# liayan/Legion-1

Measured on AMD Instinct MI355X. Metric: sampled edges/s + feature GB/s, 3-hop GraphSAGE ogbn-papers100M at 1/2/4/8 GPU, higher is better.
Workload: dtype int32 ids / f32 rows (verbatim copy)

## Files before the change

### legion-1_amd/csrc/internal.h

```cpp
#pragma once
#include <hip/hip_runtime.h>
#include <cstdint>
#include <cstdio>
#include <cstdlib>
#include <iostream>
#include <string>
#include <vector>

#include "../../include/legion_amd.h"
#include "audit.h"

namespace legion {

void report_error(const char* file, int line, const char* msg, bool hip_failure);
bool error_pending();
bool error_is_fatal();
int64_t ipc_max_bytes();
bool ipc_size_ok(int64_t bytes, const char* who);
bool ipc_export_ok(const void* ptr, const char* who);
int64_t shard_chunk_bytes();
inline void check(hipError_t e, const char* file, int line)
{
    if (e != hipSuccess) report_error(file, line, hipGetErrorString(e), true);
}
#define HIP_CHECK(expr) ::legion::check((expr), __FILE__, __LINE__)
#define HIP_CHECK_LAST() ::legion::check(hipGetLastError(), __FILE__, __LINE__)
#define LEGION_ARG_ERROR(msg) ::legion::report_error(__FILE__, __LINE__, (msg), false)

std::ostream& log_out();
FILE* log_file();

int physical_device(int logical);
bool is_remote_device(int logical);
struct DeviceGuard {
    int prev = -1, prev_logical = -1;
    explicit DeviceGuard(int logical);
    ~DeviceGuard();
};

int chunk_shift(int64_t unit_bytes, int min_shift);
inline int chunk_count(int64_t n, int shift) { return n > 0 ? (int)(((n - 1) >> shift) + 1) : 1; }
template <typename T>
struct ChunkList {
    std::vector<T*> chunks;
    bool imported = false;
    T* at(int q) const { return q >= 0 && q < (int)chunks.size() ? chunks[q] : nullptr; }
    bool complete(size_t n) const { for (T* p : chunks) if (!p) return false; return chunks.size() == n; }
    void release();
    int export_chunk(int dev, int q, void* handle64, const char* who) const;
    int import_chunk(int q, const void* handle64, int64_t floor_bytes, int open_dev, const char* who);
};
template <typename T> void upload_table(int viewer, const std::vector<T*>& h, T**& tab, bool realloc, const char* what);

typedef unsigned long long pos_t;
constexpr int kPosShift = 32;
constexpr uint32_t kProvisional = 0x80000000u, kPosValueMask = 0x7FFFFFFFu;
constexpr uint32_t kEpochTop = 0xFFFFFFFFu, kSerialLimit = 0xFFFFFFF0u;
__host__ __device__ inline pos_t pos_entry(uint32_t epoch, uint32_t value) { return ((pos_t)epoch << kPosShift) | (pos_t)value; }
#ifndef LEGION_KTILE
#define LEGION_KTILE 1024
#endif
constexpr int kTile = LEGION_KTILE;
constexpr int kBlock = 256;
static_assert(kTile >= kBlock && kTile <= 2048 && (kTile & (kTile - 1)) == 0, "LEGION_KTILE: a power of two in [256, 2048] (k_sample stages 16 bytes of row descriptor per slot in static LDS)");
#ifndef LEGION_NARROW_SLOTS
#define LEGION_NARROW_SLOTS (256 * 1024)
#endif
constexpr int kTileNarrow = kBlock;
constexpr int64_t kNarrowSlots = LEGION_NARROW_SLOTS;
static_assert(kTileNarrow <= kTile, "one pow_tab of kTile entries serves both tile sizes");
constexpr int64_t sampler_tile_of(int64_t slots_bound) { return slots_bound <= kNarrowSlots ? kTileNarrow : kTile; }
constexpr int64_t sampler_max_tiles(int64_t max_slots)
{
    const int64_t wide = (max_slots + kTile - 1) / kTile, narrow_slots = max_slots < kNarrowSlots ? max_slots : kNarrowSlots;
    const int64_t narrow = (narrow_slots + kTileNarrow - 1) / kTileNarrow;
    return wide > narrow ? wide : narrow;
}
constexpr int kDistinctMaxFanout = 64;
constexpr int32_t kSamplingReplace = 0, kSamplingDistinct = 1, kSamplingWeighted = 2;
struct AliasEntry { uint32_t thr; int32_t alias_id; };
static_assert(sizeof(AliasEntry) == 8, "one 8-byte probe per weighted draw");
constexpr int32_t kAliasHubDegree = 256;
constexpr int kMaxChunks = 2048;
static_assert(kMaxChunks % kBlock == 0 && kMaxChunks >= 256 * 8, "kMaxChunks: a multiple of the workgroup size, >= 256 CUs x 8 workgroups");
constexpr int ilog2_c(int v) { return v <= 1 ? 0 : 1 + ilog2_c(v >> 1); }
constexpr int kMaxParts = LEGION_MAX_DEVICE;

struct ServeModes {
    bool agg_last_hop = false;
    int32_t agg_norm = 0;
    int32_t sampling = 0;
    bool seeded = false;
    uint32_t seed = 0;
    int32_t lp_draw = 0;
    bool weighted_distinct = false;
    bool operator==(const ServeModes& o) const { return agg_last_hop == o.agg_last_hop && agg_norm == o.agg_norm && sampling == o.sampling && seeded == o.seeded && seed == o.seed && lp_draw == o.lp_draw && weighted_distinct == o.weighted_distinct; }
};
bool serve_modes_from_env(ServeModes& m, std::string& why);
bool serve_modes_resolve_lp_draw(ServeModes& m, bool lp_lists, int32_t raw_batch_size, std::string& why);
bool serve_modes_fit_fanout(const ServeModes& m, const int32_t* fanout, int32_t hops, std::string& why);
void runner_set_lists_verbatim(Runner* r, bool verbatim);
void ipc_env_publish_modes(IPCEnv* e, const ServeModes& m);

constexpr int kModes = 3;
static_assert(LEGION_TRAINMODE == 0 && LEGION_VALIDMODE == 1 && LEGION_TESTMODE == 2, "seed sets are indexed by mode");
struct BuildInfoSeedFields {
    const int32_t* LegionBuildInfo::*num;
    const int32_t* const* LegionBuildInfo::*ids;
    const int32_t* const* LegionBuildInfo::*labels;
};
constexpr BuildInfoSeedFields kBuildInfoSeeds[kModes] = {
    {&LegionBuildInfo::training_set_num, &LegionBuildInfo::training_set_ids, &LegionBuildInfo::training_labels},
    {&LegionBuildInfo::validation_set_num, &LegionBuildInfo::validation_set_ids, &LegionBuildInfo::validation_labels},
    {&LegionBuildInfo::testing_set_num, &LegionBuildInfo::testing_set_ids, &LegionBuildInfo::testing_labels}};

constexpr uint32_t kP31 = 2147483647u;
constexpr uint32_t kA = 48271u;

__host__ __device__ inline uint32_t mulmod31(uint32_t a, uint32_t b)
{
    uint64_t p = (uint64_t)a * (uint64_t)b;
    uint32_t r = (uint32_t)(p & kP31) + (uint32_t)(p >> 31);
    r = (r & kP31) + (r >> 31);
    return r >= kP31 ? r - kP31 : r;
}

__host__ __device__ inline uint32_t powmod31(uint32_t base, uint64_t e)
{
    uint32_t r = 1;
    while (e) {
        if (e & 1) r = mulmod31(r, base);
        base = mulmod31(base, base);
        e >>= 1;
    }
    return r;
}

__host__ __device__ inline uint32_t mix32(uint32_t z)
{
    z ^= z >> 16; z *= 0x7feb352du; z ^= z >> 15; z *= 0x846ca68bu; z ^= z >> 16;
    return z;
}
constexpr uint32_t kShuffleTag = 0x53485546u, kDrawTag = 0x44524157u, kGolden = 0x9E3779B9u;
constexpr uint32_t kLpPosTag = 0x4C50504Fu, kLpNegTag = 0x4C504E45u;
__host__ __device__ inline uint32_t seeded_shuffle_key(uint32_t seed, uint32_t round) { return mix32(mix32(seed ^ kShuffleTag) ^ round); }
__host__ __device__ inline uint32_t seeded_draw_key(uint32_t seed, uint32_t round) { return mix32(mix32(seed ^ kDrawTag) ^ round); }
__host__ __device__ inline uint32_t seeded_draw_word(uint32_t seeded, uint32_t draw_key, int32_t counter) { return seeded ? mix32(draw_key ^ (uint32_t)counter) : 0u; }
__host__ __device__ inline uint32_t seeded_stream_seed(uint32_t w) { return 1u + w % 2147483646u; }
__host__ __device__ inline uint32_t seeded_perm(uint32_t g, uint32_t n, uint32_t ks)
{
    if (n <= 1) return g;
    uint32_t b = 0;
    while (b < 32 && ((n - 1) >> b)) b++;
    const uint32_t h = (b + 1) >> 1, m = (1u << h) - 1u;
    uint32_t rk[4];
    for (uint32_t q = 0; q < 4; q++) rk[q] = mix32(ks + q * kGolden);
    uint32_t x = g;
    do {
        uint32_t L = x >> h, R = x & m;
        for (uint32_t q = 0; q < 4; q++) { const uint32_t t = L ^ (mix32(R ^ rk[q]) & m); L = R; R = t; }
        x = (L << h) | R;
    } while (x >= n);
    return x;
}

struct FastDiv {
    uint32_t d = 1, m = 0, s = 0;
    FastDiv() = default;
    explicit FastDiv(uint32_t div);
};

struct CsrTables {
    const int64_t* indptr;
    const int32_t* indices;
    const int64_t* const* frag_indptr;
    const int32_t* const* frag_indices;
    int32_t ip_nch, ix_nch, row_shift, edge_shift;
    int32_t partition_count;
    const int8_t* topo_owner;
    const int32_t* topo_row;
};

struct BatchCtl {
    int32_t counter;
    uint32_t epoch;
    uint32_t draw;
    uint32_t seeded;
    uint32_t draw_key;
};

struct HopState {
    int32_t edge_base, node_base, n_edges, n_nodes, in_off, n_in, slots, pad;
};

struct SamplerBuffers {
    int32_t* sampled_ids;
    int32_t* agg_src_ids;
    int32_t* agg_src_off;
    int32_t* agg_dst_off;
    int32_t* nc;
    int32_t* ec;
    pos_t* pos_map;
    const BatchCtl* ctl;
    int32_t* cand;
    int32_t* aux;
    int32_t* aux_next;
    int32_t next_count;
    int32_t aux_cap;
    int32_t ids_cap;
    int32_t V;
    bool aux_prepared;
    int32_t* tile_edge;
    int32_t* tile_node;
    int2* tile_pre;
    int2* chunk_tot;
    HopState* hop_state;
    unsigned long long* edge_access_time;
};

struct LpDrawArgs {
    int32_t k = 0;
    int32_t V = 0;
    CsrTables csr = {};
};
void launch_seed(hipStream_t s, int32_t* batch_ids, int32_t* labels, int32_t batch_size, int32_t size, int32_t counter,
                 const int32_t* all_ids, const int32_t* all_labels, int32_t total_cap, pos_t* pos_map,
                 uint32_t epoch, BatchCtl* ctl, bool self_driven, int32_t* nc, int32_t* ec, int32_t* aux_next,
                 int32_t f_next, int32_t aux_cap, uint32_t seeded = 0, uint32_t draw_key = 0, const LpDrawArgs* lp = nullptr);
void launch_set_cursor(hipStream_t s, BatchCtl* ctl, int32_t counter, uint32_t epoch, uint32_t seeded = 0, uint32_t draw_key = 0);
void launch_shuffle_seeds(hipStream_t s, const int32_t* ids, const int32_t* labels, int32_t n, uint32_t ks, int32_t* out_ids, int32_t* out_labels);
void launch_shuffle_triples(hipStream_t s, const int32_t* ids, const int32_t* labels, int32_t n, int32_t k, uint32_t ks, int32_t* out_ids, int32_t* out_labels);
void launch_advance(hipStream_t s, BatchCtl* ctl);
int sampler_cu_count();
void warm_static_tables();
void launch_sample_hop(hipStream_t s, const CsrTables& csr, const SamplerBuffers& b, int32_t count, int32_t op_id,
                       int32_t hops, int32_t slots_bound, bool is_presc, int32_t sampling = kSamplingReplace, const AliasEntry* alias = nullptr,
                       const float* weights = nullptr);
void launch_check_weights(hipStream_t s, const float* w, int64_t E, unsigned long long* bad);
void launch_build_alias(hipStream_t s, const int64_t* indptr, const int32_t* indices, const float* w, int32_t V, int64_t E, double* p, AliasEntry* table);
void launch_weighted_probe(hipStream_t s, const int32_t* row, const int32_t* hop, const int32_t* slot, const int32_t* deg, const uint32_t* word,
                           int32_t* k, uint32_t* ub, int32_t n);
void launch_weighted_distinct_probe(hipStream_t s, const int32_t* row, const int32_t* hop, const int32_t* col, const uint32_t* word, const float* w,
                                    uint32_t* u, double* key, int32_t n);
void launch_find_feat(hipStream_t s, const int32_t* sampled_ids, int32_t* cache_offset, const int32_t* nc,
                      int32_t op_id, const int32_t* feat_map, int32_t bound);
void launch_find_topo(hipStream_t s, const int32_t* input_ids, int8_t* part_index, int32_t* part_offset,
                      int32_t batch_size, const int8_t* topo_owner, const int32_t* topo_row);
struct GatherArgs {
    const float* table;
    const float* const* shard_tab;
    int32_t chunk_shift, nchunks;
    const int32_t* feat_map;
    const float** row_ptr;
    int32_t cache_capacity;
    int32_t F;
    int32_t table_pitch, shard_pitch;
    int32_t total_num_nodes;
    const int32_t* sampled_ids;
    const int32_t* nc;
    float* dst;
    int32_t off_idx, size_idx;
    int32_t dst_rows;
    int32_t* rows_seen;
    int32_t* hit_stats;
    int32_t rows_hint;
    bool table_on_host;
    bool row_ptr_ready;
};
void launch_gather(hipStream_t s, const GatherArgs& a, int32_t rows_bound);
void launch_gather_sum(hipStream_t s, const GatherArgs& a, const int32_t* cand, int32_t cand_cap, const int32_t* ec, int32_t hops,
                       int32_t f, int32_t runs_bound, const float* wdraw = nullptr);
struct AggNormArgs {
    const int32_t* nc;
    const int32_t* ec;
    int32_t hops, f;
    const int32_t* cand;
    int32_t cand_cap;
    const int32_t* src_off;
    int32_t ids_cap;
    int32_t* out_deg;
    int32_t* chunk_cnt;
    float* wdraw;
};
void launch_agg_norm_weights(hipStream_t s, const AggNormArgs& a, int32_t slots_bound, int32_t edges_bound);
constexpr int kRowsSeenAll = LEGION_MAX_HOPS + 1;
constexpr int kRowsSeenAggIn = LEGION_MAX_HOPS + 2;
constexpr int kRowsSeenAggRuns = LEGION_MAX_HOPS + 3;
constexpr int kRowsSeenWords = LEGION_MAX_HOPS + 4;
void launch_exchange_plan(hipStream_t s, const GatherArgs& g, int32_t me, int32_t Kg, int32_t* slot, int32_t* counts,
                          int32_t* req_row, int32_t* req_dst, int32_t rows_bound);
void launch_exchange_rows(hipStream_t s, bool scatter, const float* const* shard_chunks, int32_t chunk_shift, const int32_t* list,
                          int32_t n, int32_t F, int32_t shard_pitch, const float* in, float* out, int32_t out_rows);
void launch_hotness(hipStream_t s, const int32_t* ids, const int32_t* nc, int32_t hops, unsigned long long* access,
                    int32_t* max_ids, int32_t bound);
void launch_rng_probe(hipStream_t s, const int32_t* idx, const int32_t* deg, int32_t* k, int32_t n);
void launch_distinct_probe(hipStream_t s, const int32_t* row, const int32_t* hop, const int32_t* deg, int32_t f, int32_t* pos, int32_t n);
void launch_seeded_rng_probe(hipStream_t s, uint32_t w, const int32_t* idx, const int32_t* deg, int32_t* k, int32_t n);
void launch_seeded_distinct_probe(hipStream_t s, uint32_t w, const int32_t* row, const int32_t* hop, const int32_t* deg, int32_t f, int32_t* pos, int32_t n);
void launch_perm_probe(hipStream_t s, uint32_t ks, int32_t n, int32_t* out);
void launch_lp_draw_probe(hipStream_t s, uint32_t w, const int32_t* src, const int32_t* deg, int32_t V, int32_t* rho, int32_t* neg, int32_t n);
void launch_aggregate_access(hipStream_t s, unsigned long long* agg, const unsigned long long* add, int32_t n);
void launch_iota(hipStream_t s, int32_t* out, int32_t n);
void launch_build_feat_map(hipStream_t s, int32_t* feat_map, const int32_t* QF, int32_t capacity, int32_t Kg, int32_t V);
void launch_build_topo_map(hipStream_t s, int8_t* owner, int32_t* row, const int32_t* QT, int32_t capacity, int32_t Kg,
                           int32_t Ki, int32_t V);
void launch_fill_i32(hipStream_t s, int32_t* p, int32_t v, int64_t n);
void launch_fill_i8(hipStream_t s, int8_t* p, int8_t v, int64_t n);
void launch_feat_fill_up(hipStream_t s, int32_t row0, int32_t rows, int32_t F, int32_t chunk_pitch, int32_t table_pitch, float* chunk,
                         const float* table, const int32_t* QF, int32_t Kg, int32_t Ki, int32_t V);
void launch_copy_rows_pitched(hipStream_t s, float* dst, int32_t dst_pitch, const float* src, int32_t src_pitch, int32_t F, int64_t rows);
void launch_neighbor_count(hipStream_t s, const int32_t* QT, int32_t Kg, int32_t Ki, int32_t capacity, int32_t V,
                           const int64_t* indptr, int64_t* count_out);
void launch_topo_fill_up(hipStream_t s, const int32_t* QT, int32_t Kg, int32_t Ki, int32_t capacity, int32_t V,
                         const int64_t* indptr, const int32_t* indices, const int64_t* frag_indptr,
                         int32_t* const* frag_chunks, int32_t edge_shift);
void launch_chunk_ends(hipStream_t s, const int64_t* frag_indptr, int32_t capacity, int32_t edge_shift, int32_t nch, int64_t* ends);
void launch_edge_mem(hipStream_t s, const int32_t* order, uint64_t* edge_mem, int32_t V, const int64_t* indptr);
void launch_topo_transactions(hipStream_t s, const int32_t* order, const uint64_t* hot, uint64_t* out, int32_t V, const int64_t* indptr);
void sort_by_hotness_desc(hipStream_t s, unsigned long long* keys, int32_t* ids, int32_t n);
void inclusive_scan_u64(hipStream_t s, const uint64_t* in, uint64_t* out, int32_t n);
void inclusive_scan_i64(hipStream_t s, const int64_t* in, int64_t* out, int32_t n);

}

struct PeerExchange;
struct GPUMemoryPool {
    int32_t pipeline_depth = LEGION_PIPELINE_DEPTH;
    int32_t current_pipe = 0, iter = 0, mode = 0, op_id = 0;
    int32_t device_id = -1;
    bool owns_scratch = false;
    int32_t V = 0, batch_size = 0, hops = 0, num_ids = 0;
    int32_t fanout[LEGION_MAX_HOPS] = {0};
    int32_t max_slots = 0, max_tiles = 0;
    int32_t feature_rows = 0;
    legion::pos_t* pos_map = nullptr;
    uint32_t batch_serial = 0;
    legion::BatchCtl* ctl = nullptr;
    int32_t* rows_seen = nullptr;
    int32_t* rows_seen_dev = nullptr;
    bool capturing = false;
    bool ctl_synced = false;
    int32_t ctl_counter = 0;
    int32_t* cand = nullptr;
    legion::ServeModes modes;
    std::vector<int32_t*> cand_pipe;
    int32_t sampled_hop = 0;
    bool sampled_presc = false;
    uint32_t levels_gathered = 0;
    uint32_t round = 0;
    int32_t* shuf_ids = nullptr;
    int32_t* shuf_labels = nullptr;
    int32_t shuf_cap = 0, shuf_n = 0;
    const int32_t* shuf_src = nullptr;
    bool shuf_valid = false, shuf_file_order = false;
    bool seed_reads_shuffle = false;
    GPUGraphStorage* lp_graph = nullptr;
    std::vector<int32_t*> agg_out_deg, agg_chunk_cnt;
    std::vector<float*> agg_wdraw;
    int32_t* aux2[2] = {nullptr, nullptr};
    int32_t aux_ready_hop = 0, aux_ready_count = 0;
    int32_t* tile_edge = nullptr;
    int32_t* tile_node = nullptr;
    int2* tile_pre = nullptr;
    int2* chunk_tot = nullptr;
    legion::HopState* hop_state = nullptr;
    int32_t* cache_search_buffer = nullptr;
    const float** row_ptr = nullptr;
    PeerExchange* peer_exchange = nullptr;
    int32_t* agg_src_ids = nullptr;
    int8_t* tmp_part_ind = nullptr;
    int32_t* tmp_part_off = nullptr;
    std::vector<float*> float_features;
    std::vector<int32_t*> labels, node_counter, edge_counter, sampled_ids, agg_src_off, agg_dst_off;
    int32_t bound_n = 0;
    int32_t bound_nodes = 0;
    int32_t level_bound[LEGION_MAX_HOPS + 1] = {0};
    explicit GPUMemoryPool(int32_t depth);
};
namespace legion {
bool pool_apply_modes(GPUMemoryPool* p, const ServeModes& wanted, const char* who);
}

struct GPUGraphStorage {
    int32_t partition_count = 0;
    int32_t node_num = 0;
    int64_t edge_num = 0, cache_edge_num = 0;
    int64_t* csr_node_index_cpu = nullptr;
    int32_t* csr_dst_node_ids_cpu = nullptr;
    std::vector<int64_t*> replica_indptr;
    std::vector<int32_t*> replica_indices;
    std::vector<legion::AliasEntry*> alias;
    std::vector<float*> weights;
    bool retain_weights = false;
    int32_t csr_location = LEGION_LOC_HOST_PINNED;
    bool owns_csr = false;
    struct Fragment {
        int32_t rows = 0;
        int64_t edges = 0;
        legion::ChunkList<int64_t> ip;
        legion::ChunkList<int32_t> ix;
        bool complete = false;
    };
    std::vector<Fragment> frag;
    int32_t row_shift = 27, edge_shift = 28;
    std::vector<std::vector<bool>> view;
    std::vector<void**> d_frag_tab;
    int32_t ip_nch = 1, ix_nch = 1;
};

struct GPUNodeStorage {
    int32_t partition_count = 0, total_num_nodes = 0, float_attr_len = 0;
    float* float_attrs = nullptr;
    int32_t float_attr_pitch = 0;
    std::vector<float*> replica_attrs;
    int32_t replica_pitch = 0;
    int32_t features_location = LEGION_LOC_HOST_PINNED;
    bool owns_features = false;
    struct SeedSet { int32_t num = 0; int32_t* ids = nullptr; int32_t* labels = nullptr; };
    std::vector<SeedSet> seeds[legion::kModes];
    const SeedSet& seed_set(int32_t mode, int32_t p) const
    {
        static const SeedSet none;
        return mode >= 0 && mode < legion::kModes && p >= 0 && p < (int32_t)seeds[mode].size() ? seeds[mode][p] : none;
    }
};

struct CacheController {
    int32_t device_idx = 0, device_count = 1, total_num_nodes = 0, train_step = 0;
    unsigned long long* node_access_time = nullptr;
    unsigned long long* edge_access_time = nullptr;
    int32_t iter = 0, max_ids = 0;
    int32_t* d_max_ids = nullptr;
    int32_t node_capacity = 0, edge_capacity = 0;
    int32_t* feat_map = nullptr;
    int8_t* topo_owner = nullptr;
    int32_t* topo_row = nullptr;
    int32_t* d_global_count = nullptr;
    int32_t find_iter = 0;
    int32_t* hit_stats = nullptr;
    int32_t* hit_stats_dev = nullptr;
    hipEvent_t hit_ev[2] = {nullptr, nullptr};
    bool hit_ev_armed[2] = {false, false};
    int32_t hit_samples = 0;
    double last_hit_rate = -1.0;
};

struct GPUCache {
    int32_t device_count = 0;
    std::vector<CacheController*> ctl;
    std::vector<int32_t*> QF, QT;
    std::vector<unsigned long long*> AF, AT;
    int Kc = 1, Kg = 1;
    std::vector<int32_t> node_capacity, edge_capacity;
    std::vector<double> alpha;
    int64_t cache_memory = 0;
    int32_t int_attr_len = 0, float_attr_len = 0, train_step = 0;
    std::vector<legion::ChunkList<float>> shards;
    std::vector<float**> d_shard_tab;
    std::vector<int32_t> chunk_shift, nchunks;
    int32_t shard_pitch = 0;
    bool is_presc = true;
    bool capacity_forced = false;
    int32_t forced_node_capacity = 0, forced_edge_capacity = 0;
};
```

### legion-1_amd/csrc/sampler.hip

```cpp
#include "internal.h"
#include "draws.h"
#include "launch.h"
#include <mutex>

#include "audit_hooks.h"

namespace legion {

__device__ inline int32_t lp_pos(const CsrTables& c, uint32_t w, uint32_t i, int32_t src)
{
    const int64_t* ip = c.indptr + src;
    const int32_t* rowp;
    const int8_t owner = c.topo_owner ? c.topo_owner[src] : (int8_t)-1;
    int64_t start;
    if (owner >= 0) {
        const int32_t row = c.topo_row[src];
        ip = c.frag_indptr[owner * c.ip_nch + (row >> c.row_shift)] + (row & ((1 << c.row_shift) - 1));
        start = ip[0];
        rowp = c.frag_indices[owner * c.ix_nch + (int32_t)(start >> c.edge_shift)] + (start & ((1ll << c.edge_shift) - 1));
    } else {
        start = ip[0];
        rowp = c.indices + start;
    }
    const int32_t d = (int32_t)(ip[1] - start);
    if (d <= 0) return src;
    const int32_t pos = rowp[lp_rho(w, i, src, d)];
    return pos < 0 ? src : pos;
}

template <bool SELF, bool LP>
__global__ __launch_bounds__(kBlock) void k_seed(int32_t* __restrict__ batch_ids, int32_t* __restrict__ labels,
                                                 int32_t batch_size, int32_t size, int32_t counter,
                                                 const int32_t* __restrict__ all_ids,
                                                 const int32_t* __restrict__ all_labels, int32_t total_cap,
                                                 pos_t* __restrict__ pos_map, uint32_t epoch,
                                                 BatchCtl* __restrict__ ctl, int32_t* __restrict__ nc,
                                                 int32_t* __restrict__ ec, int32_t* __restrict__ aux_next,
                                                 int32_t f_next, int32_t aux_cap, uint32_t seeded, uint32_t draw_key, LpDrawArgs lp)
{
    int32_t idx = threadIdx.x + blockDim.x * blockIdx.x;
    if (SELF) {
        counter = ctl->counter;
        epoch = ctl->epoch;
        const int64_t done = (int64_t)batch_size * counter;
        size = (done + batch_size >= total_cap) ? (int32_t)max((int64_t)0, min((int64_t)batch_size, (int64_t)total_cap - done)) : batch_size;
    } else if (idx == 0) {
        ctl->counter = counter;
        ctl->epoch = epoch;
        ctl->draw = seeded_draw_word(seeded, draw_key, counter);
        ctl->seeded = seeded;
        ctl->draw_key = draw_key;
    }
    if (idx < size) {
        int32_t g = size * counter + idx;
        if (g >= total_cap) {
            batch_ids[idx] = -1;
            labels[idx] = -1;
        } else {
            int32_t src_id, label;
            if constexpr (LP) {
                const int32_t q = (idx >= lp.k) + (idx >= 2 * lp.k), i = idx - q * lp.k;
                const int32_t gs = g - q * lp.k;
                const uint32_t w = SELF ? ctl->draw : seeded_draw_word(seeded, draw_key, counter);
                src_id = all_ids[gs];
                label = -1;
                if (q == 0) label = all_labels[gs];
                else if (q == 1) src_id = lp_pos(lp.csr, w, (uint32_t)i, src_id);
                else src_id = lp_neg(w, (uint32_t)i, src_id, lp.V);
            } else {
                src_id = all_ids[g % total_cap];
            }
            batch_ids[idx] = src_id;
            const pos_t mine = pos_entry(epoch, (uint32_t)idx);
            pos_t cur = pos_map[src_id];
            while ((uint32_t)(cur >> kPosShift) != epoch || cur < mine) {
                const pos_t seen = atomicCAS(pos_map + src_id, cur, mine);
                if (seen == cur) break;
                cur = seen;
            }
            if constexpr (LP) labels[idx] = label;
            else labels[idx] = all_labels[g % total_cap];
        }
    }
    if (idx < LEGION_COUNTER_WORDS) {
        constexpr int seeds = legion_idx_level_size(0);
        int32_t nv = 0;
        if (idx == LEGION_NC_TOTAL || idx == LEGION_NC_NEXT_INPUTS || idx == seeds) nv = size;
        nc[idx] = nv;
        ec[idx] = 0;
    }
    const int64_t n_init = min((int64_t)max(size, 0) * f_next, (int64_t)aux_cap);
    for (int64_t i = idx; i < n_init; i += (int64_t)gridDim.x * blockDim.x) aux_next[i] = -1;
}
__global__ void k_fill_aux(const int32_t* __restrict__ nc, int32_t count, int32_t* __restrict__ aux, int32_t aux_cap)
{
    const int64_t n = min((int64_t)nc[LEGION_NC_NEXT_INPUTS] * count, (int64_t)aux_cap);
    for (int64_t i = threadIdx.x + (int64_t)blockDim.x * blockIdx.x; i < n; i += (int64_t)gridDim.x * blockDim.x) aux[i] = -1;
}
__global__ void k_set_cursor(BatchCtl* ctl, int32_t counter, uint32_t epoch, uint32_t seeded, uint32_t draw_key)
{
    ctl->counter = counter; ctl->epoch = epoch;
    ctl->draw = seeded_draw_word(seeded, draw_key, counter); ctl->seeded = seeded; ctl->draw_key = draw_key;
}
__global__ void k_advance(BatchCtl* ctl)
{
    const int32_t counter = ctl->counter + 1;
    ctl->counter = counter; ctl->epoch -= 1;
    ctl->draw = seeded_draw_word(ctl->seeded, ctl->draw_key, counter);
}

__global__ __launch_bounds__(kBlock) void k_shuffle_seeds(const int32_t* __restrict__ ids, const int32_t* __restrict__ labels, int32_t n, uint32_t ks,
                                                          int32_t* __restrict__ out_ids, int32_t* __restrict__ out_labels)
{
    const int32_t g = threadIdx.x + blockDim.x * blockIdx.x;
    if (g >= n) return;
    const uint32_t p = seeded_perm((uint32_t)g, (uint32_t)n, ks);
    out_ids[g] = ids[p];
    out_labels[g] = labels[p];
}

__global__ __launch_bounds__(kBlock) void k_shuffle_triples(const int32_t* __restrict__ ids, const int32_t* __restrict__ labels, int32_t n, int32_t k, uint32_t ks,
                                                            int32_t* __restrict__ out_ids, int32_t* __restrict__ out_labels)
{
    const int32_t g = threadIdx.x + blockDim.x * blockIdx.x;
    if (g >= n) return;
    const int32_t b = g / (3 * k), r = g - b * 3 * k, q = r / k, i = r - q * k;
    const uint32_t t = seeded_perm((uint32_t)(b * k + i), (uint32_t)(n / 3), ks);
    const int32_t from = (int32_t)(t / (uint32_t)k) * 3 * k + q * k + (int32_t)(t % (uint32_t)k);
    out_ids[g] = ids[from];
    out_labels[g] = labels[from];
}


struct SampleArgs {
    CsrTables csr;
    const int32_t* sampled_ids;
    const int32_t* agg_src_ids;
    const int32_t* nc;
    const int32_t* ec;
    pos_t* pos_map;
    int32_t* cand;
    int32_t* aux;
    int32_t* tile_edge;
    unsigned long long* edge_access_time;
    const BatchCtl* ctl;
    const uint32_t* pow_tab;
    uint32_t a_tile;
    uint32_t a_step;
    FastDiv fdiv;
    int32_t count;
    int32_t op_id;
    int32_t window;
    int32_t prefilter_from_op;
    union {
        const AliasEntry* alias;
        const float* weights;
    };
};

__device__ inline int32_t claim_slot(const SampleArgs& a, uint32_t epoch, int32_t dst, int32_t idx)
{
    const pos_t prov0 = pos_entry(epoch, kProvisional);
    const pos_t mine = prov0 | (pos_t)(uint32_t)idx;
    pos_t cur = (a.op_id < a.prefilter_from_op) ? ~(pos_t)0 : a.pos_map[dst];
    if (cur > mine) {
        const pos_t old = atomicMin(a.pos_map + dst, mine);
        if (old > mine) {
            if ((uint32_t)(old >> kPosShift) == epoch) a.aux[(uint32_t)old & kPosValueMask] = -2 - idx;
            cur = mine;
        } else {
            cur = old;
        }
    }
    if (cur < prov0) return (int32_t)((uint32_t)cur & kPosValueMask);
    if (cur < mine) return -2 - (int32_t)((uint32_t)cur & kPosValueMask);
    return -1;
}

template <int TILE, bool PRESC, bool PARTITIONED, bool DISTINCT, bool WEIGHTED>
__global__ __launch_bounds__(kBlock) void k_sample(SampleArgs a)
{
    static_assert(!(WEIGHTED && PARTITIONED), "weighted draws read the whole CSR");
    constexpr bool STREAM = !DISTINCT && !WEIGHTED;
    __shared__ const int32_t* s_row[TILE + 2];
    __shared__ int32_t s_deg[TILE + 2];
    __shared__ int32_t s_src[TILE + 2];
    __shared__ int32_t s_cnt[kBlock / 64];
    __shared__ int32_t s_pick[DISTINCT ? TILE + 2 * kDistinctMaxFanout : 1];

    const int32_t N = a.nc[LEGION_NC_NEXT_INPUTS];
    const int32_t f = a.count;
    const int32_t total = N * f;
    const int32_t* __restrict__ input = (a.op_id == 2) ? a.sampled_ids : a.agg_src_ids + a.ec[LEGION_EC_INPUT_OFF];
    const int32_t n_tiles = (total + TILE - 1) / TILE;
    const int tid = threadIdx.x;
    const uint32_t epoch = a.ctl->epoch;
    const uint32_t draw = a.ctl->draw;

    if ((int32_t)blockIdx.x >= n_tiles) return;

    uint32_t x[TILE / kBlock];
    if constexpr (STREAM) {
        uint32_t base = mulmod31(powmod31(a.a_tile, (uint64_t)blockIdx.x), seeded_stream_seed(draw));
#pragma unroll
        for (int s = 0; s < TILE / kBlock; s++) x[s] = mulmod31(base, a.pow_tab[tid + kBlock * s]);
    }

    for (int32_t tile = blockIdx.x; tile < n_tiles; tile += gridDim.x) {
        const int32_t tile_start = tile * TILE;
        const int32_t tile_end = min(tile_start + TILE, total);
        const int32_t i0 = (int32_t)fdiv((uint32_t)tile_start, a.fdiv);
        const int32_t i_last = (int32_t)fdiv((uint32_t)(tile_end - 1), a.fdiv);
        const int32_t nrows = i_last - i0 + 1;

        for (int32_t r = tid; r < nrows; r += kBlock) {
            const int32_t src = input[i0 + r];
            const int32_t* rowp = nullptr;
            int32_t deg = -1;
            if (src >= 0) {
                const int64_t* ip = a.csr.indptr + src;
                const int32_t* ix = a.csr.indices;
                int8_t owner = -1;
                if (PARTITIONED && !PRESC) owner = a.csr.topo_owner[src];
                if (owner >= 0) {
                    const int32_t row = a.csr.topo_row[src];
                    ip = a.csr.frag_indptr[owner * a.csr.ip_nch + (row >> a.csr.row_shift)] + (row & ((1 << a.csr.row_shift) - 1));
                    const int64_t start = ip[0];
                    ix = a.csr.frag_indices[owner * a.csr.ix_nch + (int32_t)(start >> a.csr.edge_shift)];
                    rowp = ix + (start & ((1ll << a.csr.edge_shift) - 1));
                    deg = (int32_t)(ip[1] - start);
                } else {
                    const int64_t start = ip[0];
                    rowp = ix + start;
                    deg = (int32_t)(ip[1] - start);
                }
            }
            s_row[r] = rowp;
            s_deg[r] = deg;
            s_src[r] = src;
        }
        if constexpr (DISTINCT && !WEIGHTED) {
            const uint32_t hop = (uint32_t)a.op_id >> 1;
            for (int32_t p = tid; p < nrows * f; p += kBlock) {
                const uint32_t rr = fdiv((uint32_t)p, a.fdiv);
                s_pick[p] = (int32_t)distinct_u(distinct_key((uint32_t)i0 + rr, hop, draw), (uint32_t)p - rr * (uint32_t)f);
            }
        }
        __syncthreads();
        if constexpr (DISTINCT && !WEIGHTED) {
            for (int32_t r = tid; r < nrows; r += kBlock)
                if (s_deg[r] > f) distinct_resolve(s_pick + r * f, s_deg[r], f);
            __syncthreads();
        }
        if constexpr (DISTINCT && WEIGHTED) {
            const uint32_t hop = (uint32_t)a.op_id >> 1;
            for (int32_t r = wave_id(); r < nrows; r += kBlock / 64) {
                const int32_t d = s_deg[r];
                if (d <= 0) continue;
                const int32_t got = weighted_distinct_resolve(s_pick + r * f, a.weights + (s_row[r] - a.csr.indices), d, f,
                                                              weighted_distinct_key((uint32_t)(i0 + r), hop, draw));
                if (lane_id() == 0) s_deg[r] = got;
            }
            __syncthreads();
        }

        int32_t cnt = 0;
#pragma unroll
        for (int s = 0; s < TILE / kBlock; s++) {
            const int32_t idx = tile_start + tid + kBlock * s;
            int32_t dst = -1, known = -1, j = 0, r = 0;
            if (idx < tile_end) {
                const uint32_t i = fdiv((uint32_t)idx, a.fdiv);
                j = idx - (int32_t)i * f;
                r = (int32_t)i - i0;
                const int32_t deg = s_deg[r];
                if (j < deg) {
                    if constexpr (DISTINCT && WEIGHTED) dst = s_row[r][s_pick[r * f + j]];
                    else if constexpr (DISTINCT) dst = s_row[r][deg <= f ? j : s_pick[r * f + j]];
                    else if constexpr (WEIGHTED) {
                        const uint32_t key = weighted_key(i, (uint32_t)a.op_id >> 1, draw);
                        const int32_t* col = s_row[r] + weighted_column(key, (uint32_t)j, deg);
                        const AliasEntry e = a.alias[col - a.csr.indices];
                        const int32_t own = *col;
                        dst = weighted_ub(key, (uint32_t)j) < e.thr ? own : e.alias_id;
                    }
                    else dst = s_row[r][sample_index(x[s], deg)];
                    if (dst < 0) dst = -1;
                }
            }
            int32_t dup = 0;
            for (int d = 1; d <= a.window; d++) {
                const int32_t o = __shfl_up(dst, d);
                if (d <= j && d <= lane_id() && o == dst) dup = d;
            }
            if (dst >= 0) {
                if (PRESC) atomicAdd(a.edge_access_time + s_src[r], 1ull);
                if (dup) known = -2 - (idx - dup);
                else known = claim_slot(a, epoch, dst, idx);
                cnt++;
            }
            if (idx < tile_end) {
                a.cand[idx] = dst;
                if (dst < 0) a.aux[idx] = 0;
                else if (known != -1) a.aux[idx] = known;
            }
        }
        for (int o = 32; o > 0; o >>= 1) cnt += __shfl_down(cnt, o);
        if (lane_id() == 0) s_cnt[wave_id()] = cnt;
        __syncthreads();
        if (tid == 0) {
            int32_t t = 0;
#pragma unroll
            for (int w = 0; w < kBlock / 64; w++) t += s_cnt[w];
            a.tile_edge[tile] = t;
        }
        if constexpr (STREAM) {
#pragma unroll
            for (int s = 0; s < TILE / kBlock; s++) x[s] = mulmod31(x[s], a.a_step);
        }
        __syncthreads();
    }
}

constexpr int32_t kWinBase = 0x40000000;

__device__ inline int32_t enc_win(int32_t r) { return -2 - (kWinBase + r); }
__device__ inline bool is_win(int32_t v) { return v <= -2 - kWinBase; }
__device__ inline int32_t win_rank(int32_t v) { return -2 - v - kWinBase; }

__host__ __device__ inline FastDiv make_fastdiv(uint32_t div)
{
    FastDiv f;
    f.d = div ? div : 1;
    if (f.d == 1) { f.m = 0; f.s = 0; return f; }
    uint32_t l = 0;
    while ((1ull << l) < f.d) l++;
    f.m = (uint32_t)(((1ull << (31 + l)) / f.d) + 1ull);
    f.s = 31 + l;
    return f;
}

template <int TILE>
__global__ __launch_bounds__(kBlock) void k_mark(const int32_t* __restrict__ nc, const int32_t* __restrict__ ec,
                                                 int32_t count, int32_t* __restrict__ aux, const int32_t* __restrict__ tile_edge,
                                                 int32_t* __restrict__ tile_node, int2* __restrict__ tile_pre,
                                                 int2* __restrict__ chunk_tot, HopState* __restrict__ hs)
{
    constexpr int S = TILE / kBlock, W = kBlock / 64;
    __shared__ int32_t s_c[S * W];
    const int32_t total = nc[LEGION_NC_NEXT_INPUTS] * count;
    const int32_t n_tiles = (total + TILE - 1) / TILE;
    const int lane = lane_id(), wave = wave_id();
    const unsigned long long lt = (1ull << lane) - 1ull;
    if (blockIdx.x == 0 && threadIdx.x == 0) {
        HopState h;
        h.edge_base = ec[LEGION_EC_TOTAL]; h.node_base = nc[LEGION_NC_TOTAL]; h.n_edges = 0; h.n_nodes = 0;
        h.in_off = ec[LEGION_EC_INPUT_OFF]; h.n_in = nc[LEGION_NC_NEXT_INPUTS]; h.slots = total; h.pad = 0;
        *hs = h;
    }
    const int32_t T = (n_tiles + (int32_t)gridDim.x - 1) / (int32_t)gridDim.x;
    const int32_t t0 = (int32_t)blockIdx.x * T, t1 = min(t0 + T, n_tiles);
    if (t0 >= n_tiles) return;
    int32_t nxt[S];
#pragma unroll
    for (int s = 0; s < S; s++) {
        const int64_t idx = (int64_t)t0 * TILE + threadIdx.x + kBlock * s;
        nxt[s] = idx < total ? aux[idx] : 0;
    }
    int32_t te_next = threadIdx.x == 0 ? tile_edge[t0] : 0, run_e = 0, run_n = 0;
    for (int32_t tile = t0; tile < t1; tile++) {
        bool win[S];
        int32_t rk[S];
        const int32_t te = te_next;
#pragma unroll
        for (int s = 0; s < S; s++) {
            const int32_t idx = tile * TILE + threadIdx.x + kBlock * s;
            win[s] = idx < total && nxt[s] == -1;
        }
        {
            const int64_t nt = (int64_t)tile + 1;
#pragma unroll
            for (int s = 0; s < S; s++) {
                const int64_t idx = nt * TILE + threadIdx.x + kBlock * s;
                nxt[s] = (nt < t1 && idx < total) ? aux[idx] : 0;
            }
            if (threadIdx.x == 0 && nt < t1) te_next = tile_edge[nt];
        }
#pragma unroll
        for (int s = 0; s < S; s++) {
            const unsigned long long b = __ballot(win[s]);
            rk[s] = __popcll(b & lt);
            if (lane == 0) s_c[s * W + wave] = __popcll(b);
        }
        __syncthreads();
        int32_t run = 0, before[S];
#pragma unroll
        for (int q = 0; q < S * W; q++) {
#pragma unroll
            for (int s = 0; s < S; s++)
                if (q == s * W + wave) before[s] = run;
            run += s_c[q];
        }
#pragma unroll
        for (int s = 0; s < S; s++)
            if (win[s]) aux[tile * TILE + threadIdx.x + kBlock * s] = enc_win(before[s] + rk[s]);
        if (threadIdx.x == 0) {
            tile_node[tile] = run;
            tile_pre[tile] = make_int2(run_e, run_n);
            run_e += te; run_n += run;
        }
        __syncthreads();
    }
    if (threadIdx.x == 0) chunk_tot[blockIdx.x] = make_int2(run_e, run_n);
}

__device__ inline void apply_update_counter(int32_t* nc, int32_t* ec, int32_t op_id, int32_t hops, int32_t n_nodes,
                                            int32_t n_edges)
{
    const int32_t hh = op_id / 2;
    const int off = legion_idx_level_offset(hh), size = legion_idx_level_size(hh);
    nc[LEGION_NC_TOTAL] += n_nodes;
    nc[off] = nc[off - LEGION_LEVEL_WORDS] + nc[size - LEGION_LEVEL_WORDS];
    nc[size] = n_nodes;
    if (hh == hops) nc[legion_idx_nodes_through(hh)] = nc[off] + nc[size];
    nc[LEGION_NC_HOP_NEW] = 0;
    nc[LEGION_NC_NEXT_INPUTS] = n_edges;
    const int32_t before = hh == 1 ? hh : hh - 1;
    ec[legion_idx_edges_through(hh)] = ec[legion_idx_edges_through(before)] + n_edges;
    ec[LEGION_EC_INPUT_OFF] = ec[LEGION_EC_TOTAL];
    ec[LEGION_EC_TOTAL] += n_edges;
    ec[LEGION_EC_HOP] = 0;
}

struct WriteArgs {
    HopState* hs;
    int32_t* nc;
    int32_t* ec;
    int32_t hops;
    const int32_t* cand;
    const int32_t* aux;
    const int32_t* tile_edge;
    const int32_t* tile_node;
    int32_t* sampled_ids;
    int32_t* agg_src_ids;
    int32_t* agg_src_off;
    int32_t* agg_dst_off;
    pos_t* pos_map;
    FastDiv fdiv;
    int32_t op_id;
    const BatchCtl* ctl;
    int32_t last_hop;
    const int2* tile_pre;
    const int2* chunk_tot;
    int32_t mark_grid;
    int32_t* aux_next;
    int32_t next_count;
    int32_t aux_cap;
    int32_t ids_cap;
    int32_t V;
};


template <int TILE>
__global__ __launch_bounds__(kBlock) void k_write(WriteArgs a)
{
    constexpr int S = TILE / kBlock, W = kBlock / 64;
    __shared__ int2 s_chunk[kMaxChunks];
    __shared__ int32_t s_e[S * W];
    __shared__ int2 s_scan[W];
    __shared__ uint32_t s_div_t[3];
    constexpr int PER = kMaxChunks / kBlock;
    const int32_t q0 = (int32_t)threadIdx.x * PER;
    int2 v[PER];
#pragma unroll
    for (int u = 0; u < PER; u++) v[u] = a.chunk_tot[q0 + u];
    int32_t c[S], so[S];
#pragma unroll
    for (int s = 0; s < S; s++) {
        const int64_t idx = (int64_t)blockIdx.x * TILE + threadIdx.x + kBlock * s;
        c[s] = idx < a.aux_cap ? a.cand[idx] : -1;
        so[s] = idx < a.aux_cap ? a.aux[idx] : 0;
    }
    int2 own = a.tile_pre[blockIdx.x];
    int32_t tile_e = a.tile_edge[blockIdx.x];
    const HopState h = *a.hs;
    const uint32_t epoch = a.ctl->epoch;
    const int32_t total = h.slots;
    const int32_t n_tiles = (total + TILE - 1) / TILE;
    const int lane = lane_id(), wave = wave_id();
    const unsigned long long lt = (1ull << lane) - 1ull;
    if (n_tiles == 0) {
        if (blockIdx.x == 0 && threadIdx.x == 0) apply_update_counter(a.nc, a.ec, a.op_id, a.hops, 0, 0);
        return;
    }
    if ((int32_t)blockIdx.x >= n_tiles) return;
    const int32_t T = (n_tiles + a.mark_grid - 1) / a.mark_grid;
    if (threadIdx.x == 0) {
        const FastDiv f = make_fastdiv((uint32_t)T);
        s_div_t[0] = f.d; s_div_t[1] = f.m; s_div_t[2] = f.s;
    }
    const int32_t n_chunks = (n_tiles + T - 1) / T;
    {
        int32_t se = 0, sn = 0;
#pragma unroll
        for (int u = 0; u < PER; u++) {
            if (q0 + u >= n_chunks) v[u] = make_int2(0, 0);
            se += v[u].x; sn += v[u].y;
        }
        int32_t ie = se, in = sn;
        for (int o = 1; o < 64; o <<= 1) {
            const int32_t ue = __shfl_up(ie, o), un = __shfl_up(in, o);
            if (lane >= o) { ie += ue; in += un; }
        }
        if (lane == 63) s_scan[wave] = make_int2(ie, in);
        __syncthreads();
        int32_t run_e = ie - se, run_n = in - sn;
#pragma unroll
        for (int w = 0; w < W; w++)
            if (w < wave) { run_e += s_scan[w].x; run_n += s_scan[w].y; }
#pragma unroll
        for (int u = 0; u < PER; u++) {
            if (q0 + u < n_chunks) s_chunk[q0 + u] = make_int2(run_e, run_n);
            run_e += v[u].x; run_n += v[u].y;
        }
        __syncthreads();
    }
    FastDiv div_t;
    div_t.d = s_div_t[0]; div_t.m = s_div_t[1]; div_t.s = s_div_t[2];
    auto nodes_before = [&](int32_t t, int32_t pre_n_in_chunk) { return s_chunk[fdiv((uint32_t)t, div_t)].y + pre_n_in_chunk; };

    for (int32_t tile = blockIdx.x; tile < n_tiles; tile += gridDim.x) {
        const bool first = tile == (int32_t)blockIdx.x;
        if (!first) { own = a.tile_pre[tile]; tile_e = a.tile_edge[tile]; }
        const int2 own_chunk = s_chunk[fdiv((uint32_t)tile, div_t)];
        const int32_t pre_e = own_chunk.x + own.x, pre_n = own_chunk.y + own.y;
        const int32_t ebase = h.edge_base + pre_e;
        const int32_t nbase = h.node_base + pre_n;
        int32_t dpos[S], w[S], re[S], wpre[S];
        const int32_t* __restrict__ pre_n_of = reinterpret_cast<const int32_t*>(a.tile_pre) + 1;
#pragma unroll
        for (int s = 0; s < S; s++) {
            const int32_t idx = tile * TILE + threadIdx.x + kBlock * s;
            if (!first) {
                c[s] = (idx < total) ? a.cand[idx] : -1;
                so[s] = (idx < total) ? a.aux[idx] : 0;
            } else if (idx >= total) { c[s] = -1; so[s] = 0; }
        }
#pragma unroll
        for (int s = 0; s < S; s++) {
            dpos[s] = 0; w[s] = -1;
            if (c[s] == -1) continue;
            const int32_t idx = tile * TILE + threadIdx.x + kBlock * s;
            const int32_t i = (int32_t)fdiv((uint32_t)idx, a.fdiv);
            dpos[s] = (a.op_id == 2) ? (int32_t)((uint32_t)a.pos_map[a.sampled_ids[i]] & kPosValueMask) : a.agg_src_off[h.in_off + i];
            wpre[s] = 0;
            if (so[s] < -1 && !is_win(so[s])) { w[s] = -2 - so[s]; so[s] = a.aux[w[s]]; wpre[s] = pre_n_of[2 * (w[s] / TILE)]; }
        }
#pragma unroll
        for (int s = 0; s < S; s++)
            while (w[s] >= 0 && so[s] < -1 && !is_win(so[s])) { w[s] = -2 - so[s]; so[s] = a.aux[w[s]]; wpre[s] = pre_n_of[2 * (w[s] / TILE)]; }
#pragma unroll
        for (int s = 0; s < S; s++) {
            const unsigned long long be = __ballot(c[s] != -1);
            re[s] = __popcll(be & lt);
            if (lane == 0) s_e[s * W + wave] = __popcll(be);
        }
        __syncthreads();
        if (tile == n_tiles - 1 && threadIdx.x == 0) {
            const int32_t n_edges = pre_e + tile_e, n_nodes = pre_n + a.tile_node[tile];
            a.hs->n_edges = n_edges;
            a.hs->n_nodes = n_nodes;
            apply_update_counter(a.nc, a.ec, a.op_id, a.hops, n_nodes, n_edges);
        }
#pragma unroll
        for (int s = 0; s < S; s++) {
            if (c[s] == -1) continue;
            int32_t pe = 0;
            for (int q = 0; q < s * W + wave; q++) pe += s_e[q];
            const int32_t dst = c[s];
            const int32_t e = ebase + pe + re[s];
            if (!LEGION_STORE_OK(e, a.ids_cap)) continue;
            if (!a.last_hop) a.agg_src_ids[e] = dst;
            a.agg_dst_off[e] = dpos[s];
            int32_t p = so[s];
            if (w[s] >= 0) {
                if (p < -1)
                    p = h.node_base + nodes_before(w[s] / TILE, wpre[s]) + win_rank(p);
            } else if (is_win(p)) {
                p = nbase + win_rank(p);
                if (LEGION_STORE_OK(p, a.ids_cap)) a.sampled_ids[p] = dst;
                if (!a.last_hop && LEGION_STORE_OK(dst, a.V)) a.pos_map[dst] = pos_entry(epoch, (uint32_t)p);
            }
            a.agg_src_off[e] = p;
        }
        if (a.next_count > 0) {
            const int64_t lo = min((int64_t)pre_e * a.next_count, (int64_t)a.aux_cap);
            const int64_t hi = min((int64_t)(pre_e + tile_e) * a.next_count, (int64_t)a.aux_cap);
            for (int64_t q = lo + threadIdx.x; q < hi; q += kBlock) a.aux_next[q] = -1;
        }
        __syncthreads();
    }
}

FastDiv::FastDiv(uint32_t div)
{
    d = div ? div : 1;
    if (d == 1) { m = 0; s = 0; return; }
    uint32_t l = 0;
    while ((1ull << l) < d) l++;
    m = (uint32_t)(((1ull << (31 + l)) / d) + 1ull);
    s = 31 + l;
}

int sampler_cu_count()
{
    static int cus = 0;
    if (!cus) {
        int dev = 0;
        hipDeviceProp_t p;
        if (hipGetDevice(&dev) == hipSuccess && hipGetDeviceProperties(&p, dev) == hipSuccess)
            cus = p.multiProcessorCount;
        if (cus <= 0) cus = 256;
    }
    return cus;
}

static uint32_t* pow_table()
{
    static uint32_t* tabs[64] = {nullptr};
    static std::mutex mu;
    std::lock_guard<std::mutex> lk(mu);
    int dev = 0;
    HIP_CHECK(hipGetDevice(&dev));
    if (!tabs[dev]) {
        std::vector<uint32_t> h(kTile);
        uint32_t x = 1;
        for (int m = 0; m < kTile; m++) { x = mulmod31(x, kA); h[m] = x; }
        HIP_CHECK(hipMalloc(&tabs[dev], kTile * sizeof(uint32_t)));
        HIP_CHECK(hipMemcpy(tabs[dev], h.data(), kTile * sizeof(uint32_t), hipMemcpyHostToDevice));
    }
    LEGION_AUDIT_SHARE(tabs[dev], current_logical_device());
    return tabs[dev];
}

void launch_seed(hipStream_t s, int32_t* batch_ids, int32_t* labels, int32_t batch_size, int32_t size, int32_t counter,
                 const int32_t* all_ids, const int32_t* all_labels, int32_t total_cap, pos_t* pos_map,
                 uint32_t epoch, BatchCtl* ctl, bool self_driven, int32_t* nc, int32_t* ec, int32_t* aux_next,
                 int32_t f_next, int32_t aux_cap, uint32_t seeded, uint32_t draw_key, const LpDrawArgs* lp)
{
    const int32_t bound = self_driven ? batch_size : size;
    int blocks = bound > 0 ? (bound - 1) / kBlock + 1 : 1;
    LEGION_AUDIT_LAUNCH(s, "k_seed", LEGION_AW(batch_ids), LEGION_AW(labels), LEGION_AW(pos_map), LEGION_AW(ctl), LEGION_AW(nc), LEGION_AW(ec), LEGION_AW(aux_next), LEGION_AL(all_ids), LEGION_AL(all_labels));
    const LpDrawArgs a = lp ? *lp : LpDrawArgs{};
    auto* k = lp ? (self_driven ? k_seed<true, true> : k_seed<false, true>) : (self_driven ? k_seed<true, false> : k_seed<false, false>);
    k<<<blocks, kBlock, 0, s>>>(batch_ids, labels, batch_size, size, counter, all_ids, all_labels, total_cap, pos_map, epoch, ctl, nc, ec, aux_next, f_next, aux_cap, seeded, draw_key, a);
    HIP_CHECK_LAST();
}
void launch_set_cursor(hipStream_t s, BatchCtl* ctl, int32_t counter, uint32_t epoch, uint32_t seeded, uint32_t draw_key)
{
    LEGION_AUDIT_LAUNCH(s, "k_set_cursor", LEGION_AW(ctl));
    k_set_cursor<<<1, 1, 0, s>>>(ctl, counter, epoch, seeded, draw_key);
    HIP_CHECK_LAST();
}
void launch_shuffle_seeds(hipStream_t s, const int32_t* ids, const int32_t* labels, int32_t n, uint32_t ks, int32_t* out_ids, int32_t* out_labels)
{
    if (n <= 0) return;
    LEGION_AUDIT_LAUNCH(s, "k_shuffle_seeds", LEGION_AW(out_ids), LEGION_AW(out_labels), LEGION_AL(ids), LEGION_AL(labels));
    k_shuffle_seeds<<<(n + kBlock - 1) / kBlock, kBlock, 0, s>>>(ids, labels, n, ks, out_ids, out_labels);
    HIP_CHECK_LAST();
}
void launch_shuffle_triples(hipStream_t s, const int32_t* ids, const int32_t* labels, int32_t n, int32_t k, uint32_t ks, int32_t* out_ids, int32_t* out_labels)
{
    if (n <= 0 || k <= 0 || n % (3 * k) != 0) return;
    LEGION_AUDIT_LAUNCH(s, "k_shuffle_triples", LEGION_AW(out_ids), LEGION_AW(out_labels), LEGION_AL(ids), LEGION_AL(labels));
    k_shuffle_triples<<<(n + kBlock - 1) / kBlock, kBlock, 0, s>>>(ids, labels, n, k, ks, out_ids, out_labels);
    HIP_CHECK_LAST();
}
void launch_advance(hipStream_t s, BatchCtl* ctl)
{
    LEGION_AUDIT_LAUNCH(s, "k_advance", LEGION_AW(ctl));
    k_advance<<<1, 1, 0, s>>>(ctl);
    HIP_CHECK_LAST();
}
void warm_static_tables() { (void)pow_table(); (void)sampler_cu_count(); }

template <int TILE>
static void launch_sample_hop_t(hipStream_t s, const CsrTables& csr, const SamplerBuffers& b, int32_t count, int32_t op_id,
                       int32_t hops, int32_t slots_bound, bool is_presc, int32_t sampling, const AliasEntry* alias, const float* weights)
{
    const int max_tiles = (slots_bound + TILE - 1) / TILE;
    constexpr int wg_per_cu = TILE == kTile ? 4 : 8;
    const int grid = std::min(grid_for(max_tiles, 1, wg_per_cu), kMaxChunks);
    if (!b.aux_prepared) {
        LEGION_AUDIT_LAUNCH(s, "k_fill_aux", LEGION_AW(b.aux), LEGION_AL(b.nc));
        k_fill_aux<<<grid_for(slots_bound, kBlock * 4), kBlock, 0, s>>>(b.nc, count, b.aux, b.aux_cap);
        HIP_CHECK_LAST();
    }
    SampleArgs a;
    a.csr = csr;
    a.sampled_ids = b.sampled_ids; a.agg_src_ids = b.agg_src_ids; a.nc = b.nc; a.ec = b.ec;
    a.pos_map = b.pos_map; a.cand = b.cand; a.aux = b.aux; a.tile_edge = b.tile_edge;
    a.edge_access_time = b.edge_access_time;
    a.ctl = b.ctl;
    a.pow_tab = pow_table();
    a.a_tile = powmod31(kA, TILE);
    a.a_step = powmod31(kA, (uint64_t)TILE * (uint64_t)grid);
    a.fdiv = FastDiv((uint32_t)count);
    a.count = count; a.op_id = op_id;
    a.window = std::min(count - 1, 8);
    a.prefilter_from_op = 4;
    const bool wdistinct = sampling == kSamplingWeighted && weights;
    a.alias = sampling == kSamplingWeighted ? alias : nullptr;
    if (wdistinct) a.weights = weights;
    const bool part = csr.topo_owner != nullptr;
    LEGION_AUDIT_LAUNCH(s, "k_sample", LEGION_AW(a.pos_map), LEGION_AW(a.cand), LEGION_AW(a.aux), LEGION_AW(a.tile_edge), LEGION_AW(a.edge_access_time), LEGION_AL(a.sampled_ids), LEGION_AL(a.agg_src_ids), LEGION_AL(a.nc), LEGION_AL(a.ec), LEGION_AL(a.ctl), LEGION_AL(a.pow_tab), LEGION_AL(csr.frag_indptr), LEGION_AL(csr.frag_indices), LEGION_AL(csr.topo_owner), LEGION_AL(csr.topo_row), LEGION_AR(csr.indptr), LEGION_AR(csr.indices), LEGION_AL(a.alias));
    if (wdistinct) {
        if (is_presc) k_sample<TILE, true, false, true, true><<<grid, kBlock, 0, s>>>(a);
        else k_sample<TILE, false, false, true, true><<<grid, kBlock, 0, s>>>(a);
    }
    else if (sampling == kSamplingWeighted) {
        if (is_presc) k_sample<TILE, true, false, false, true><<<grid, kBlock, 0, s>>>(a);
        else k_sample<TILE, false, false, false, true><<<grid, kBlock, 0, s>>>(a);
    }
    else if (sampling == kSamplingDistinct) {
        if (is_presc) k_sample<TILE, true, false, true, false><<<grid, kBlock, 0, s>>>(a);
        else if (part) k_sample<TILE, false, true, true, false><<<grid, kBlock, 0, s>>>(a);
        else k_sample<TILE, false, false, true, false><<<grid, kBlock, 0, s>>>(a);
    }
    else if (is_presc) k_sample<TILE, true, false, false, false><<<grid, kBlock, 0, s>>>(a);
    else if (part) k_sample<TILE, false, true, false, false><<<grid, kBlock, 0, s>>>(a);
    else k_sample<TILE, false, false, false, false><<<grid, kBlock, 0, s>>>(a);
    HIP_CHECK_LAST();
    LEGION_AUDIT_LAUNCH(s, "k_mark", LEGION_AW(b.aux), LEGION_AW(b.tile_node), LEGION_AW(b.tile_pre), LEGION_AW(b.chunk_tot), LEGION_AW(b.hop_state), LEGION_AL(b.nc), LEGION_AL(b.ec), LEGION_AL(b.tile_edge));
    k_mark<TILE><<<grid, kBlock, 0, s>>>(b.nc, b.ec, count, b.aux, b.tile_edge, b.tile_node, b.tile_pre, b.chunk_tot, b.hop_state);
    HIP_CHECK_LAST();
    WriteArgs w;
    w.hs = b.hop_state; w.nc = b.nc; w.ec = b.ec; w.hops = hops; w.cand = b.cand; w.aux = b.aux; w.ctl = b.ctl; w.tile_edge = b.tile_edge; w.tile_node = b.tile_node;
    w.sampled_ids = b.sampled_ids; w.agg_src_ids = b.agg_src_ids; w.agg_src_off = b.agg_src_off;
    w.agg_dst_off = b.agg_dst_off; w.pos_map = b.pos_map; w.fdiv = a.fdiv; w.op_id = op_id; w.last_hop = (op_id / 2 == hops) ? 1 : 0;
    w.aux_next = b.aux_next; w.next_count = b.next_count; w.aux_cap = b.aux_cap; w.ids_cap = b.ids_cap; w.V = b.V;
    w.tile_pre = b.tile_pre; w.chunk_tot = b.chunk_tot; w.mark_grid = grid;
    const int wgrid = grid_for(max_tiles, 1, 8);
    LEGION_AUDIT_LAUNCH(s, "k_write", LEGION_AW(w.hs), LEGION_AW(w.nc), LEGION_AW(w.ec), LEGION_AW(w.sampled_ids), LEGION_AW(w.agg_src_ids), LEGION_AW(w.agg_src_off), LEGION_AW(w.agg_dst_off), LEGION_AW(w.pos_map), LEGION_AW(w.aux_next), LEGION_AL(w.cand), LEGION_AL(w.aux), LEGION_AL(w.tile_edge), LEGION_AL(w.tile_node), LEGION_AL(w.tile_pre), LEGION_AL(w.chunk_tot), LEGION_AL(w.ctl));
    k_write<TILE><<<wgrid, kBlock, 0, s>>>(w);
    HIP_CHECK_LAST();
}

void launch_sample_hop(hipStream_t s, const CsrTables& csr, const SamplerBuffers& b, int32_t count, int32_t op_id,
                       int32_t hops, int32_t slots_bound, bool is_presc, int32_t sampling, const AliasEntry* alias, const float* weights)
{
    if (count <= 0 || slots_bound <= 0) { LEGION_ARG_ERROR("GPU_Random_Sampling: empty hop"); return; }
    const bool distinct = sampling == kSamplingDistinct;
    if (sampling == kSamplingWeighted && (!alias || csr.topo_owner)) { LEGION_ARG_ERROR("GPU_Random_Sampling: weighted sampling (GPUMemoryPool_SetSampling) draws from the whole CSR's alias table: the graph has none (GPUGraphStorage_SetEdgeWeights)"); return; }
    if (distinct && count > kDistinctMaxFanout) { LEGION_ARG_ERROR("GPU_Random_Sampling: distinct sampling (GPUMemoryPool_SetSampleDistinct) takes a fan-out of at most 64: k_sample stages the picks of a tile's rows in static LDS"); return; }
    if (weights && sampling == kSamplingWeighted && count > kDistinctMaxFanout) { LEGION_ARG_ERROR("GPU_Random_Sampling: weighted sampling without replacement (GPUMemoryPool_SetWeightedDistinct) takes a fan-out of at most 64: k_sample keeps a row's best picks one per lane and stages them in static LDS"); return; }
    if (sampler_tile_of(slots_bound) == kTileNarrow) launch_sample_hop_t<kTileNarrow>(s, csr, b, count, op_id, hops, slots_bound, is_presc, sampling, alias, weights);
    else launch_sample_hop_t<kTile>(s, csr, b, count, op_id, hops, slots_bound, is_presc, sampling, alias, weights);
}

}
```

Before: 6.730 billion.

## Prefetch next tile's candidates and skip seed pos_map lookups when seeds are unique

The compaction kernel now loads the next grid-stride tile's cand/aux values and tile prefix data before processing the current tile. This overlaps those global loads with the current tile's work. Separately, the seed-init kernel records in a new dup_epoch control field whether any seed id repeated in this epoch. When no seed repeats, the first hop uses the seed index directly instead of gathering pos_map[sampled_ids[i]]. The cost is extra registers for the prefetched values, and correctness relies on dup_epoch being visible across kernels and starting from a value that never equals the current epoch.

```diff
diff --git a/legion-1_amd/csrc/internal.h b/legion-1_amd/csrc/internal.h
--- a/legion-1_amd/csrc/internal.h
+++ b/legion-1_amd/csrc/internal.h
@@ -187,6 +187,7 @@
     uint32_t draw;
     uint32_t seeded;
     uint32_t draw_key;
+    uint32_t dup_epoch;
 };
 
 struct HopState {
diff --git a/legion-1_amd/csrc/sampler.hip b/legion-1_amd/csrc/sampler.hip
--- a/legion-1_amd/csrc/sampler.hip
+++ b/legion-1_amd/csrc/sampler.hip
@@ -73,11 +73,14 @@
             batch_ids[idx] = src_id;
             const pos_t mine = pos_entry(epoch, (uint32_t)idx);
             pos_t cur = pos_map[src_id];
+            bool repeated = (uint32_t)(cur >> kPosShift) == epoch;
             while ((uint32_t)(cur >> kPosShift) != epoch || cur < mine) {
                 const pos_t seen = atomicCAS(pos_map + src_id, cur, mine);
                 if (seen == cur) break;
                 cur = seen;
-            }
+                repeated = true;
+            }
+            if (repeated) ctl->dup_epoch = epoch;
             if constexpr (LP) labels[idx] = label;
             else labels[idx] = all_labels[g % total_cap];
         }
@@ -485,6 +488,7 @@
     int32_t tile_e = a.tile_edge[blockIdx.x];
     const HopState h = *a.hs;
     const uint32_t epoch = a.ctl->epoch;
+    const bool seeds_repeat = a.ctl->dup_epoch == epoch;
     const int32_t total = h.slots;
     const int32_t n_tiles = (total + TILE - 1) / TILE;
     const int lane = lane_id(), wave = wave_id();
@@ -531,7 +535,6 @@
 
     for (int32_t tile = blockIdx.x; tile < n_tiles; tile += gridDim.x) {
         const bool first = tile == (int32_t)blockIdx.x;
-        if (!first) { own = a.tile_pre[tile]; tile_e = a.tile_edge[tile]; }
         const int2 own_chunk = s_chunk[fdiv((uint32_t)tile, div_t)];
         const int32_t pre_e = own_chunk.x + own.x, pre_n = own_chunk.y + own.y;
         const int32_t ebase = h.edge_base + pre_e;
@@ -541,10 +544,7 @@
 #pragma unroll
         for (int s = 0; s < S; s++) {
             const int32_t idx = tile * TILE + threadIdx.x + kBlock * s;
-            if (!first) {
-                c[s] = (idx < total) ? a.cand[idx] : -1;
-                so[s] = (idx < total) ? a.aux[idx] : 0;
-            } else if (idx >= total) { c[s] = -1; so[s] = 0; }
+            if (first && idx >= total) { c[s] = -1; so[s] = 0; }
         }
 #pragma unroll
         for (int s = 0; s < S; s++) {
@@ -552,13 +552,25 @@
             if (c[s] == -1) continue;
             const int32_t idx = tile * TILE + threadIdx.x + kBlock * s;
             const int32_t i = (int32_t)fdiv((uint32_t)idx, a.fdiv);
-            dpos[s] = (a.op_id == 2) ? (int32_t)((uint32_t)a.pos_map[a.sampled_ids[i]] & kPosValueMask) : a.agg_src_off[h.in_off + i];
+            dpos[s] = (a.op_id == 2) ? (seeds_repeat ? (int32_t)((uint32_t)a.pos_map[a.sampled_ids[i]] & kPosValueMask) : i) : a.agg_src_off[h.in_off + i];
             wpre[s] = 0;
             if (so[s] < -1 && !is_win(so[s])) { w[s] = -2 - so[s]; so[s] = a.aux[w[s]]; wpre[s] = pre_n_of[2 * (w[s] / TILE)]; }
         }
 #pragma unroll
         for (int s = 0; s < S; s++)
             while (w[s] >= 0 && so[s] < -1 && !is_win(so[s])) { w[s] = -2 - so[s]; so[s] = a.aux[w[s]]; wpre[s] = pre_n_of[2 * (w[s] / TILE)]; }
+        const int32_t nt = tile + (int32_t)gridDim.x;
+        int32_t cn[S], son[S], te_n = 0;
+        int2 own_n = make_int2(0, 0);
+        if (nt < n_tiles) {
+#pragma unroll
+            for (int s = 0; s < S; s++) {
+                const int32_t idx = nt * TILE + threadIdx.x + kBlock * s;
+                cn[s] = (idx < total) ? a.cand[idx] : -1;
+                son[s] = (idx < total) ? a.aux[idx] : 0;
+            }
+            own_n = a.tile_pre[nt]; te_n = a.tile_edge[nt];
+        }
 #pragma unroll
         for (int s = 0; s < S; s++) {
             const unsigned long long be = __ballot(c[s] != -1);
@@ -599,6 +611,11 @@
             for (int64_t q = lo + threadIdx.x; q < hi; q += kBlock) a.aux_next[q] = -1;
         }
         __syncthreads();
+        if (nt < n_tiles) {
+#pragma unroll
+            for (int s = 0; s < S; s++) { c[s] = cn[s]; so[s] = son[s]; }
+            own = own_n; tile_e = te_n;
+        }
     }
 }
 
```

Measured after the change: 6.586 billion. 0.979x the previous value.
